# dell-research-harvard/effocr

Measured on AMD Instinct MI355X. Metric: glyph-crops/sec end-to-end (encode+kNN), 224x224 bs=1024, higher is better.
Workload: dtype bf16; 1 GPU; BASELINE configs[1]: vit_small_patch16_224 encoder (bf16 MFMA operands, fp32 accumulate/residual/LN/softmax), 1024x3x224x224 fp32 crops per GPU resident in HBM, 10000-row fp32 IndexFlatIP, k=10; seeded random-init weights; crops_per_gpu=1024, global_batch=1024, index_rows=10000, k=10, parallelism=1024 crops per GPU, weights+index replicated

## Files before the change

### effocr_amd/_lib.py

```python
import ctypes
import os
import subprocess
import threading

_HERE = os.path.dirname(os.path.abspath(__file__))
_CSRC = os.path.join(_HERE, "csrc")
SO_PATH = os.environ.get("EFFOCR_HIP_LIB") or os.path.join(_HERE, "libeffocr_hip.so")
SO_PATH_AB = os.path.join(_HERE, "libeffocr_hip_ab.so")

ABI_VERSION = 9
PREC = {"bf16": 0, "fp16": 1, "fp32": 2}
EPI = {"bias": 0, "bias_gelu": 1, "bias_resid": 2}

_lock = threading.Lock()
_lib = None
_loaded = {}


class EffOCRHipError(RuntimeError):
    pass


def build(force=False, verbose=False, ab=True):
    so = os.path.join(_HERE, "libeffocr_hip.so")
# ... 84 lines not shown
        "effocr_letterbox": (i32, [vp, i32, i32, i64, i32, i32, i32, i32, i32, i32, i32, f32p, vp]),
        "effocr_nms_workspace_bytes": (sz, [i32, i32]),
        "effocr_nms_batch_workspace_bytes": (sz, [i32, i32, i32]),
        "effocr_nms": (i32, [f32p, i32, i32, c.c_float, c.c_float, i32, i32, c.c_float, i32, f32p, vp, vp, sz, vp]),
        "effocr_nms_batch": (i32, [f32p, i32, i32, i32, c.c_float, c.c_float, i32, i32, c.c_float, i32, f32p, vp, vp, sz, vp]),
        "effocr_parse_char_boxes": (i32, [f32p, vp, i32, i32, i32, i32, i32, i32, f32p, vp, vp, vp, vp]),
        "effocr_op_linear": (i32, [i32, i32, vp, vp, f32p, f32p, vp, i32, i32, i32, vp]),
        "effocr_op_layernorm": (i32, [i32, f32p, i64, i32, f32p, f32p, c.c_float, vp, vp]),
        "effocr_op_attention": (i32, [i32, vp, vp, i32, i32, i32, vp]),
        "effocr_op_linear_blocked": (i32, [i32, i32, vp, vp, f32p, f32p, vp, i32, i32, i32, i32, vp]),
        "effocr_op_mlp_blocked": (i32, [i32, f32p, f32p, f32p, c.c_float, vp, f32p, vp, f32p, f32p, i32, i32, i32, i32, vp, sz, vp]),
        "effocr_op_mlp_ln_blocked": (i32, [i32, f32p, f32p, f32p, c.c_float, vp, f32p, vp, f32p, f32p, f32p, f32p, vp, i32, i32, i32, i32, vp, sz, vp]),
        "effocr_op_proj_mlp_blocked": (i32, [i32, f32p, vp, vp, f32p, f32p, f32p, c.c_float, vp, f32p, vp, f32p, f32p, i32, i32, i32, i32, vp, sz, vp]),
        "effocr_op_qkv_attn_blocked": (i32, [i32, vp, vp, f32p, vp, i32, i32, i32, i32, vp]),
        "effocr_op_layernorm_blocked": (i32, [i32, f32p, i64, i32, f32p, f32p, c.c_float, vp, vp]),
    }
    for name, (res, args) in sig.items():
        if os.environ.get("EFFOCR_HIP_LIB") and not hasattr(lib, name):
            def _absent(*a, _n=name, **k):
                raise EffOCRHipError(f"{_n} is not exported by the library EFFOCR_HIP_LIB points at")
            setattr(lib, name, _absent)
            continue
        fn = getattr(lib, name)
        fn.restype = res
        fn.argtypes = args
    return sig


EXPORTS = None

# ... 328 lines not shown
```

### effocr_amd/csrc/api.hip

```cpp
#include "../../include/effocr_hip.h"
#include "enc_core.hpp"


#include <math.h>
#include <algorithm>
#include <string.h>
#include <map>
#include <memory>
#include <string>
#include <vector>

namespace effocr {

namespace {

struct Param { std::string name; std::vector<int64_t> shape; int64_t numel; std::vector<float> data; bool set; };

struct VitCfg { int D, depth, heads, mlp; };
struct VitLayerOff { size_t ln1w, ln1b, qkvb, projb, ln2w, ln2b, fc1b, fc2b, qkvw, projw, fc1w, fc2w;
                     size_t qkvw_b, projw_b, fc1w_b, fc2w_b, projw_pp, fc2w_pp, projb_p, fc2b_p, qkvw_bv, qkvb_v;
                     size_t qkvw_bf, qkv_s, qkv_c, fc1w_bf, fc1_s, fc1_c; };
struct ConvSpec { std::string w, bn; int cin, cout, k, stride, pad; size_t w_off, b_off; };
struct CnxBlockOff { size_t dww, dwb, lnw, lnb, w1, b1, w2, b2, gamma; };
struct CnxStageOff { int C, Cp, depth; size_t dslnw, dslnb, dsw, dsb; std::vector<CnxBlockOff> blocks; };

}
}

using namespace effocr;

struct effocr_encoder {
  std::string arch;
  bool is_vit = false;
  int img = 224, prec = PREC_BF16, D = 0;
  std::vector<Param> params;
  std::map<std::string, int> index;
  VitCfg vit{};
  int T = 0, P = 0;
  size_t off_clspos0 = 0, off_pos = 0, off_patchb = 0, off_normw = 0, off_normb = 0, off_patchw = 0, off_patchw_b = 0;
  std::vector<VitLayerOff> layers;
  std::vector<ConvSpec> convs;
  bool is_cnx = false;
  std::vector<CnxStageOff> cnx;
  size_t cnx_stemw = 0, cnx_stemb = 0, cnx_stemlnw = 0, cnx_stemlnb = 0, cnx_headw = 0, cnx_headb = 0;
  bool is_mnv = false;
  MnvNet mnv{};
  size_t wbytes = 0;
  const char* wdev = nullptr;
  int debug = 0;
  int cls_only_last = 1;
  int mlp_stagger_min_rounds = 2;
  int mlp_tail_first = 96;
  int mlp_stagger = 2500;
  int use_projf = 1;
  int use_qkvattn = 1;
  int qa_min_batch = 1;
  int qa_hsplit = 0;
  int use_patchf = 1;
  int use_mlp = 1;
  int use_gemm3 = 1;
  int use_lnfold = 1;
  int tail_split = 1;
  int split6 = 1;
  int pair_parts = 1;
// ... 85 lines not shown
      L.fc2w_b = a.take((size_t)D * mlp * es);
      L.fc2w_pp = a.take((size_t)D * mlp * es);
      L.projw_pp = a.take((size_t)D * D * es);
      L.projb_p = a.take((size_t)D * 4);
      L.fc2b_p = a.take((size_t)D * 4);
      L.qkvw_bv = a.take((size_t)3 * D * D * es);
      L.qkvb_v = a.take((size_t)3 * D * 4);
      {
        L.qkvw_b = a.take((size_t)3 * D * D * es);
        L.projw_b = a.take((size_t)D * D * es);
        L.fc1w_b = a.take((size_t)mlp * D * es);
        L.qkvw_bf = a.take((size_t)3 * D * D * es); L.qkv_s = a.take((size_t)3 * D * 4); L.qkv_c = a.take((size_t)3 * D * 4);
        L.fc1w_bf = a.take((size_t)mlp * D * es); L.fc1_s = a.take((size_t)mlp * 4); L.fc1_c = a.take((size_t)mlp * 4);
      }
    }
  }
  e->wbytes = a.off;
}

void add_bn(effocr_encoder* e, const std::string& p, int c) {
  add_param(e, p + ".weight", {c}); add_param(e, p + ".bias", {c});
  add_param(e, p + ".running_mean", {c}); add_param(e, p + ".running_var", {c});
}

constexpr int CONV1_KPAD = 160;

void build_resnet18(effocr_encoder* e) {
  const int widths[4] = {64, 128, 256, 512};
  add_param(e, "conv1.weight", {64, 3, 7, 7});
  add_bn(e, "bn1", 64);
// ... 171 lines not shown
  float* cd = reinterpret_cast<float*>(blob.data() + c_off);
  for (int n = 0; n < N; ++n) {
    double ss = 0.0, cc = b[n];
    for (int k = 0; k < K; ++k) {
      const float v = W[(size_t)n * K + k] * gamma[k];
      wf[(size_t)n * K + k] = v;
      float r;
      if (prec == PREC_BF16) { const uint32_t u = (uint32_t)f32_to_bf16(v) << 16; memcpy(&r, &u, 4); }
      else r = (float)(_Float16)v;
      ss += (double)r;
      cc += (double)W[(size_t)n * K + k] * (double)beta[k];
    }
    sd[n] = (float)ss; cd[n] = (float)cc;
  }
  put_op_blocked(blob, w_off, wf.data(), N, K, prec);
}

void pack_vit(const effocr_encoder* e, std::vector<char>& blob) {
  const int D = e->vit.D;
  std::vector<float> cp(D);
  const auto& cls = P(e, "cls_token"); const auto& pos = P(e, "pos_embed");
  for (int d = 0; d < D; ++d) cp[d] = cls[d] + pos[d];
  put_f32(blob, e->off_clspos0, cp.data(), D);
  put_f32(blob, e->off_pos, pos.data(), pos.size());
  put_f32(blob, e->off_patchb, P(e, "patch_embed.proj.bias").data(), D);
  put_op(blob, e->off_patchw, P(e, "patch_embed.proj.weight").data(), (size_t)D * 768, e->prec);
  if (e->prec != PREC_FP32 && D % 32 == 0) put_op_blocked(blob, e->off_patchw_b, P(e, "patch_embed.proj.weight").data(), D, 768, e->prec);
  for (int i = 0; i < e->vit.depth; ++i) {
    const std::string p = "blocks." + std::to_string(i) + ".";
    const VitLayerOff& L = e->layers[i];
// ... 15 lines not shown
      put_op_blocked(blob, L.projw_pp, P(e, p + "attn.proj.weight").data(), D, D, e->prec, false, true);
      put_f32_rowperm(blob, L.projb_p, P(e, p + "attn.proj.bias").data(), D);
      put_f32_rowperm(blob, L.fc2b_p, P(e, p + "mlp.fc2.bias").data(), D);
      put_op_blocked(blob, L.qkvw_bv, P(e, p + "attn.qkv.weight").data(), 3 * D, D, e->prec, false, true, 2 * D);
      put_f32(blob, L.qkvb_v, P(e, p + "attn.qkv.bias").data(), 2 * (size_t)D);
      put_f32_rowperm(blob, L.qkvb_v + (size_t)2 * D * 4, P(e, p + "attn.qkv.bias").data() + 2 * D, D);
      {
        put_op_blocked(blob, L.qkvw_b, P(e, p + "attn.qkv.weight").data(), 3 * D, D, e->prec);
        put_op_blocked(blob, L.projw_b, P(e, p + "attn.proj.weight").data(), D, D, e->prec);
        put_op_blocked(blob, L.fc1w_b, P(e, p + "mlp.fc1.weight").data(), e->vit.mlp, D, e->prec);
        put_lnfold(blob, L.qkvw_bf, L.qkv_s, L.qkv_c, P(e, p + "attn.qkv.weight").data(), P(e, p + "attn.qkv.bias").data(),
                   P(e, p + "norm1.weight").data(), P(e, p + "norm1.bias").data(), 3 * D, D, e->prec);
        put_lnfold(blob, L.fc1w_bf, L.fc1_s, L.fc1_c, P(e, p + "mlp.fc1.weight").data(), P(e, p + "mlp.fc1.bias").data(),
                   P(e, p + "norm2.weight").data(), P(e, p + "norm2.bias").data(), e->vit.mlp, D, e->prec);
      }
    }
  }
  put_f32(blob, e->off_normw, P(e, "norm.weight").data(), D);
  put_f32(blob, e->off_normb, P(e, "norm.bias").data(), D);
}

void pack_resnet(const effocr_encoder* e, std::vector<char>& blob) {
  for (size_t ci = 0; ci < e->convs.size(); ++ci) {
    const ConvSpec& c = e->convs[ci];
    const auto& w = P(e, c.w);
    const auto& g = P(e, c.bn + ".weight"); const auto& bt = P(e, c.bn + ".bias");
    const auto& mu = P(e, c.bn + ".running_mean"); const auto& var = P(e, c.bn + ".running_var");
    const int K = c.k * c.k * c.cin;
    const int Kp = (ci == 0) ? CONV1_KPAD : K;
    float* wd = reinterpret_cast<float*>(blob.data() + c.w_off);
// ... 128 lines not shown
  }
  const int cls = prof_class(e, name);
  const size_t slot = e->prof_used++;
  const bool clk = e->prof_mode == 1 && slot < effocr_encoder::PROF_CLK_SLOTS &&
                   (e->prof_clk || hipMalloc(&e->prof_clk, effocr_encoder::PROF_CLK_SLOTS * 8192 * sizeof(unsigned long long)) == hipSuccess && hipMemset(e->prof_clk, 0, effocr_encoder::PROF_CLK_SLOTS * 8192 * sizeof(unsigned long long)) == hipSuccess);
  if (clk) (void)clock_sample(e->prof_clk + slot * 8192, s);
  (void)hipEventRecord(e->prof_pool[slot].first, s);
  const int rc = launch();
  (void)hipEventRecord(e->prof_pool[slot].second, s);
  if (clk) (void)clock_sample(e->prof_clk + slot * 8192 + 4096, s);
  e->prof_rec.push_back({cls, (int)slot});
  e->prof_work[cls] += work;
  return rc;
}

struct VitWs { size_t status, x, xn, qkv, att, h, stats, total, rows, hbytes; };
VitWs vit_ws(const effocr_encoder* e, int B) {
  const size_t M = align_up((size_t)B * e->T, 128), D = e->vit.D, es = prec_esize(e->prec);
  Alloc a; VitWs w;
  w.rows = M;
  w.status = a.take(256);
  w.x = a.take(M * D * 4);
  w.xn = a.take(M * D * es);
  w.qkv = a.take(M * 3 * D * es);
  w.att = a.take(M * D * es);
  size_t hb = M * e->vit.mlp * es, pb = (size_t)B * e->P * 768 * es;
  w.hbytes = hb > pb ? hb : pb;
  {
    const size_t cus = (size_t)device_cus(), np = M / 128, tail = np % cus;
    const size_t split = (tail && tail * 6 <= cus) ? 6 : (tail && tail * 4 <= cus) ? 4 : (tail && tail * 2 <= cus) ? 2 : 0;
// ... 12 lines not shown
  const char* wb = e->wdev;
  float* xs = reinterpret_cast<float*>(ws + w.x);
  void* xn = ws + w.xn; void* qkv = ws + w.qkv; void* att = ws + w.att; void* hb = ws + w.h;
  auto F = [&](size_t off) { return reinterpret_cast<const float*>(wb + off); };
  int rc;
  const double Md = (double)M, Dd = (double)D, Hd = (double)e->vit.mlp;
  const bool panel = e->use_panel && panel_gemm_supported(prec, 3 * D, D) && panel_gemm_supported(prec, e->vit.mlp, D);
  const bool g2 = e->use_gemm2 && gemm2_supported(prec, D, e->vit.mlp);
  const bool g2p = e->use_gemm2 && gemm2_supported(prec, D, 768);
  const bool g3all = !panel && e->use_gemm3 && gemm3_supported(prec, 3 * D, D) && gemm3_supported(prec, D, D) &&
                     gemm3_supported(prec, e->vit.mlp, D) && gemm3_supported(prec, D, e->vit.mlp);
  const int blk = (e->use_blocked && g2p && ((panel && g2) || g3all)) ? 1 : 0;
  const bool mlpf = blk && panel && e->use_mlp && mlp_fused_supported(prec, D, e->vit.mlp);
  const bool projf = mlpf && e->use_projf;
  const bool qaf = blk && panel && mlpf && qkv_attn_supported(prec, D, T) && (e->use_qkvattn == 2 || (e->use_qkvattn == 1 && (e->call_size_invariant || B >= e->qa_min_batch)));
  const bool g3 = blk && e->use_gemm3 && gemm3_supported(prec, D, e->vit.mlp);
  const bool patchf = blk && e->use_patchf && patch_embed_fused_supported(prec, D);
  if (!patchf && (rc = timed(e, "im2col_patch16", 0.0, s, [&] { return im2col_patch16(prec, x, x16, B, e->img, e->img, hb, s); }))) return rc;
  int* status = reinterpret_cast<int*>(ws + w.status);
  if (!patchf && (rc = set_cls_rows(F(e->off_clspos0), xs, B, T, D, blk, nullptr, s))) return rc;
  GemmArgs g{};
  if (patchf) {
    PatchArgs pa{};
    pa.x = x; pa.x16 = x16; pa.B = B; pa.H = e->img; pa.W = e->img; pa.Wb = wb + e->off_patchw_b; pa.bias = F(e->off_patchb); pa.pos = F(e->off_pos);
    pa.out = xs; pa.D = D; pa.P = Pn; pa.cls = F(e->off_clspos0);
    if ((rc = timed(e, "patch_embed_fused", 2.0 * B * Pn * Dd * 768.0, s, [&] { return patch_embed_fused(prec, pa, s); }))) return rc;
  } else {
  g.X = hb; g.ldx = 768; g.W = wb + e->off_patchw; g.ldw = 768; g.bias = F(e->off_patchb);
  g.out = xs; g.ldo = D; g.pos = F(e->off_pos); g.M = B * Pn; g.N = D; g.K = 768; g.P = Pn; g.blk_out = blk;
  if ((rc = timed(e, "gemm_patch_embed", 2.0 * B * Pn * Dd * 768.0, s, [&] { return g2p ? gemm2_nt(prec, EPI_PATCH, g, s) : gemm_nt(prec, EPI_PATCH, g, s); }))) return rc;
  }
  const float* cls_x = nullptr;
  bool xn_ready = false;
  for (int i = 0; i < e->vit.depth; ++i) {
    const VitLayerOff& L = e->layers[i];
    if (panel) {
      {
      PanelArgs p{};
      if (qaf) {
        if (!xn_ready && (rc = timed(e, "layernorm", 0.0, s, [&] { return layernorm_rows_blocked(prec, xs, M, D, F(L.ln1w), F(L.ln1b), 1e-6f, xn, s); }))) return rc;
        xn_ready = false;
        QkvAttnArgs q{};
        q.xn = xn; q.Wb = wb + L.qkvw_bv; q.bias = F(L.qkvb_v); q.out = att;
        q.B = B; q.T = T; q.D = D; q.rows_alloc = (int64_t)w.rows; q.hsplit = e->qa_hsplit;
        q.cls_only = (i + 1 == e->vit.depth && e->cls_only_last && projf) ? 1 : 0;
        const bool cls_k = q.cls_only && D == 384 && T > 192;
        const double qa_work = cls_k ? 2.0 * Md * 2.0 * Dd * Dd + 2.0 * (32.0 * B) * Dd * Dd + 4.0 * B * e->vit.heads * 32.0 * T * 64.0
                                     : 2.0 * Md * 3.0 * Dd * Dd + 4.0 * B * e->vit.heads * (double)T * T * 64.0;
        if ((rc = timed(e, "qkv_attn_fused", qa_work, s, [&] { return qkv_attn_fused(prec, q, s); }))) return rc;
      } else {
      p.A = xs; p.lda = D; p.gamma = F(L.ln1w); p.beta = F(L.ln1b); p.eps = 1e-6f; p.W = wb + L.qkvw; p.bias = F(L.qkvb);
      p.out = qkv; p.ldo = 3 * D; p.M = M; p.N = 3 * D; p.K = D; p.rows_padded = 1; p.debug = e->debug; p.panel_rows = e->panel_rows; p.no_tail_split = !e->tail_split;
      p.blk_a = blk; p.blk_out = blk;
      if ((rc = timed(e, "panel_ln_qkv", 2.0 * Md * 3.0 * Dd * Dd, s, [&] { return panel_gemm(prec, PRO_LN, EPI_BIAS, p, s); }))) return rc;
      if ((rc = timed(e, "attention", 4.0 * B * e->vit.heads * (double)T * T * 64.0, s, [&] { return attention(prec, qkv, att, B, T, e->vit.heads, blk, s); }))) return rc;
      }
      if (!projf) {
      p = PanelArgs{};
      p.A = att; p.lda = D; p.W = wb + L.projw; p.bias = F(L.projb); p.out = xs; p.ldo = D; p.resid = xs; p.ldr = D;
      p.M = M; p.N = D; p.K = D; p.rows_padded = 1; p.debug = e->debug; p.panel_rows = e->panel_rows; p.no_tail_split = !e->tail_split; p.blk_a = blk; p.blk_out = blk;
      if ((rc = timed(e, "panel_proj_resid", 2.0 * Md * Dd * Dd, s, [&] { return panel_gemm(prec, PRO_COPY, EPI_BIAS_RESID, p, s); }))) return rc;
      }
      }
      if (mlpf) {
        MlpArgs m{};
        m.x = xs; m.gamma = F(L.ln2w); m.beta = F(L.ln2b); m.eps = 1e-6f; m.W1b = wb + L.fc1w_b; m.b1 = F(L.fc1b);
        m.W2p = wb + L.fc2w_pp; m.b2 = F(L.fc2b_p); m.b2_logical = F(L.fc2b); m.M = M; m.D = D; m.H = e->vit.mlp; m.rows_alloc = (int)w.rows;
        m.partial = reinterpret_cast<float*>(hb); m.partial_bytes = w.hbytes; m.no_tail_split = !e->tail_split; m.no_split6 = !e->split6; m.pair = e->mlp_pair; m.no_pair_parts = !e->pair_parts; m.stagger = e->mlp_stagger; m.stagger_min_rounds = e->mlp_stagger_min_rounds; m.tail_first = e->mlp_tail_first;
        if (e->call_size_invariant) { m.no_tail_split = 1; m.pair = -1; }
        if (projf) {
          m.A = att; m.Wpp = wb + L.projw_pp; m.bp = F(L.projb_p);
          if (i + 1 == e->vit.depth && e->cls_only_last) {
            const size_t Bp = align_up((size_t)B, 128);
            float* xc = reinterpret_cast<float*>(qkv);
            void* ac = static_cast<char*>(qkv) + Bp * D * 4;
            if ((rc = timed(e, "gather_cls", 0.0, s, [&] { return gather_cls_rows_blocked(xs, att, B, T, D, xc, ac, s); }))) return rc;
            m.x = xc; m.A = ac; m.M = B; m.rows_alloc = (int)Bp;
            const double Bd = B;
            if ((rc = timed(e, "proj_mlp_cls", 4.0 * Bd * Hd * Dd + 2.0 * Bd * Dd * Dd, s, [&] { return mlp_fused(prec, m, s); }))) return rc;
            cls_x = xc;
            continue;
          }
          if (qaf && i + 1 < e->vit.depth) {
            m.xn_out = xn; m.gamma_n = F(e->layers[i + 1].ln1w); m.beta_n = F(e->layers[i + 1].ln1b);
            xn_ready = true;
          }
          if ((rc = timed(e, "proj_mlp_fused", 4.0 * Md * Hd * Dd + 2.0 * Md * Dd * Dd, s, [&] { return mlp_fused(prec, m, s); }))) return rc;
          continue;
        }
        if (qaf && i + 1 < e->vit.depth) {
          m.xn_out = xn; m.gamma_n = F(e->layers[i + 1].ln1w); m.beta_n = F(e->layers[i + 1].ln1b);
          xn_ready = true;
        }
// ... 387 lines not shown
  if (n == "debug") { enc->debug = value; return EFFOCR_OK; }
  if (n == "use_gemm2") { enc->use_gemm2 = value; return EFFOCR_OK; }
  if (n == "use_blocked") { enc->use_blocked = value; return EFFOCR_OK; }
  if (n == "tail_split") { enc->tail_split = value; return EFFOCR_OK; }
  if (n == "split6") { enc->split6 = value; return EFFOCR_OK; }
  if (n == "mlp_pair") { enc->mlp_pair = value; return EFFOCR_OK; }
  if (n == "pair_parts") { enc->pair_parts = value; return EFFOCR_OK; }
  if (n == "use_gemm3") { enc->use_gemm3 = value; return EFFOCR_OK; }
  if (n == "use_lnfold") { enc->use_lnfold = value; return EFFOCR_OK; }
  if (n == "use_mlp") { enc->use_mlp = value; return EFFOCR_OK; }
  if (n == "use_qkvattn") { enc->use_qkvattn = value; return EFFOCR_OK; }
  if (n == "qa_min_batch") { enc->qa_min_batch = value; return EFFOCR_OK; }
  if (n == "qa_hsplit") { enc->qa_hsplit = value; return EFFOCR_OK; }
  if (n == "use_patchf") { enc->use_patchf = value; return EFFOCR_OK; }
  if (n == "use_projf") { enc->use_projf = value; return EFFOCR_OK; }
  if (n == "cls_only_last") { enc->cls_only_last = value; return EFFOCR_OK; }
  if (n == "mlp_stagger_min_rounds") { enc->mlp_stagger_min_rounds = value < 1 ? 1 : value; return EFFOCR_OK; }
  if (n == "mlp_tail_first") { enc->mlp_tail_first = value < 0 ? 0 : value & ~7; return EFFOCR_OK; }
  if (n == "mlp_stagger") { enc->mlp_stagger = value < 0 ? 0 : value; return EFFOCR_OK; }
  if (n == "panel_rows") { if (value != 64 && value != 128) return fail(EFFOCR_EINVAL, "set_option: panel_rows must be 64 or 128"); enc->panel_rows = value; return EFFOCR_OK; }
  if (n == "call_size_invariant") {
    if (value != 0 && value != 1) return fail(EFFOCR_EINVAL, "set_option: call_size_invariant must be 0 or 1");
    enc->call_size_invariant = value; return EFFOCR_OK;
  }
  if (n == "chunk") { if (value < 0) return fail(EFFOCR_EINVAL, "set_option: chunk < 0"); enc->chunk = value; return EFFOCR_OK; }
  return fail(EFFOCR_EINVAL, "set_option: unknown option '" + n + "'");
}

int effocr_encoder_set_chunk(effocr_encoder_t* enc, int crops_per_chunk) {
  if (!enc || crops_per_chunk < 0) return fail(EFFOCR_EINVAL, "set_chunk: bad argument");
// ... 324 lines not shown
  a.M = m; a.D = d; a.H = h; a.rows_alloc = rows_alloc; a.partial = static_cast<float*>(scratch_dev); a.partial_bytes = scratch_bytes;
  return mlp_fused(precision, a, S(stream));
}

int effocr_op_qkv_attn_blocked(int precision, const void* xn_blk_dev, const void* wqkv_blk_dev, const float* bias_dev,
                               void* out_blk_dev, int batch, int tokens, int d, int rows_alloc, void* stream) {
  if (batch > 0 && (!xn_blk_dev || !wqkv_blk_dev || !bias_dev || !out_blk_dev))
    return fail(EFFOCR_EINVAL, "op_qkv_attn_blocked: NULL device pointer");
  if (batch < 0 || tokens < 1) return fail(EFFOCR_EINVAL, "op_qkv_attn_blocked: bad batch / tokens");
  QkvAttnArgs q{};
  q.xn = xn_blk_dev; q.Wb = wqkv_blk_dev; q.bias = bias_dev; q.out = out_blk_dev;
  q.B = batch; q.T = tokens; q.D = d; q.rows_alloc = rows_alloc;
  return qkv_attn_fused(precision, q, S(stream));
}

int effocr_op_layernorm_blocked(int out_precision, const float* x_blk_dev, int64_t rows, int d, const float* gamma_dev,
                                const float* beta_dev, float eps, void* out_blk_dev, void* stream) {
  if (rows > 0 && (!x_blk_dev || !gamma_dev || !beta_dev || !out_blk_dev)) return fail(EFFOCR_EINVAL, "op_layernorm_blocked: NULL device pointer");
  return layernorm_rows_blocked(out_precision, x_blk_dev, rows, d, gamma_dev, beta_dev, eps, out_blk_dev, S(stream));
}

int effocr_op_layernorm(int out_precision, const float* x_dev, int64_t rows, int d, const float* gamma_dev,
                        const float* beta_dev, float eps, void* out_dev, void* stream) {
  return layernorm_rows(out_precision, x_dev, rows, d, gamma_dev, beta_dev, eps, out_dev, S(stream));
}

int effocr_op_attention(int precision, const void* qkv_dev, void* out_dev, int batch, int tokens, int heads, void* stream) {
  return attention(precision, qkv_dev, out_dev, batch, tokens, heads, 0, S(stream));
}

// ... 2 lines not shown
```

### effocr_amd/csrc/kernels.hpp

```cpp
#pragma once
#include "common.hpp"

namespace effocr {

enum { PREC_BF16 = 0, PREC_FP16 = 1, PREC_FP32 = 2 };
enum { EPI_BIAS = 0, EPI_BIAS_GELU = 1, EPI_BIAS_RESID = 2, EPI_PATCH = 3,
       EPI_BIAS_SCALE_RESID = 4,
       EPI_BIAS_F32 = 5 };

static inline int prec_esize(int prec) { return prec == PREC_FP32 ? 4 : 2; }

struct GemmArgs {
  const void* X; int64_t ldx;
  const void* W; int64_t ldw;
  const float* bias;
  void* out; int64_t ldo;
  const float* resid; int64_t ldr;
  const float* pos;
  int M, N, K;
  int P;
  int blk_x;
  int blk_out;
  const void* Wblk;
  int rows_alloc;
// ... 35 lines not shown
int mlp_fused(int prec, const MlpArgs& a, hipStream_t s);

struct QkvAttnArgs {
  const void* xn;
  const void* Wb; const float* bias;
  void* out;
  int B, T, D;
  int64_t rows_alloc;
  int cls_only;
  int img0;
  int hsplit;
};
bool qkv_attn_supported(int prec, int D, int T);
int qkv_attn_fused(int prec, const QkvAttnArgs& a, hipStream_t s);

struct PatchArgs {
  const void* x; int B, H, W;
  int x16;
  const void* Wb;
  const float* bias; const float* pos;
  const float* cls;
  float* out;
  int D, P;
};
bool patch_embed_fused_supported(int prec, int D);
int patch_embed_fused(int prec, const PatchArgs& a, hipStream_t s);

enum { PRO_COPY = 0, PRO_LN = 1 };
struct PanelArgs {
  const void* A; int64_t lda;
// ... 114 lines not shown
```

### include/effocr_hip.h

```cpp
#ifndef EFFOCR_HIP_H
#define EFFOCR_HIP_H

#include <stddef.h>
#include <stdint.h>

#ifdef __cplusplus
extern "C" {
#endif

#define EFFOCR_ABI_VERSION 9

enum effocr_status {
  EFFOCR_OK = 0,
  EFFOCR_EINVAL = -1,
  EFFOCR_EUNSUPPORTED = -2,
  EFFOCR_EWORKSPACE = -3,
  EFFOCR_EHIP = -4,
  EFFOCR_ESTATE = -5,
  EFFOCR_EOVERFLOW = -6
};

enum effocr_precision {
  EFFOCR_PREC_BF16 = 0,
  EFFOCR_PREC_FP16 = 1,
// ... 114 lines not shown
                          int m, int d, int h, int rows_alloc, void* scratch_dev, size_t scratch_bytes, void* stream);
int effocr_op_mlp_ln_blocked(int precision, float* x_blk_dev, const float* gamma_dev, const float* beta_dev, float eps,
                             const void* w1_blk_dev, const float* b1_dev, const void* w2_perm_dev, const float* b2_perm_dev, const float* b2_dev,
                             const float* gamma_next_dev, const float* beta_next_dev, void* xn_blk_dev,
                             int m, int d, int h, int rows_alloc, void* scratch_dev, size_t scratch_bytes, void* stream);
int effocr_op_proj_mlp_blocked(int precision, float* x_blk_dev, const void* a_blk_dev, const void* wp_perm_dev, const float* bp_perm_dev,
                               const float* gamma_dev, const float* beta_dev, float eps, const void* w1_blk_dev, const float* b1_dev,
                               const void* w2_perm_dev, const float* b2_perm_dev, const float* b2_dev, int m, int d, int h, int rows_alloc,
                               void* scratch_dev, size_t scratch_bytes, void* stream);

int effocr_op_qkv_attn_blocked(int precision, const void* xn_blk_dev, const void* wqkv_blk_dev, const float* bias_dev,
                               void* out_blk_dev, int batch, int tokens, int d, int rows_alloc, void* stream);
int effocr_op_layernorm_blocked(int out_precision, const float* x_blk_dev, int64_t rows, int d, const float* gamma_dev,
                                const float* beta_dev, float eps, void* out_blk_dev, void* stream);

#ifdef __cplusplus
}
#endif
#endif
```

Baseline: 93720 glyph-crops/s.

## Compute last-layer CLS attention by folding K and V projections into query side

For the final ViT layer, where only the CLS token is needed, the new path skips the full K/V projection over all tokens. It computes q_cls·Wk per head (qt) and scores each token directly against the normalized input. It then forms the probability-weighted sum of inputs per head and applies Wv once per image. This removes the M×2D×D K/V GEMM on the last layer and replaces it with three custom kernels plus a specially packed weight copy. It is enabled by default for batches of at least 576 when call-size invariance is not requested, and it uses CUDA-core FMA rather than MFMA.

```diff
diff --git a/effocr_amd/_lib.py b/effocr_amd/_lib.py
--- a/effocr_amd/_lib.py
+++ b/effocr_amd/_lib.py
@@ -122,6 +122,9 @@
         "effocr_op_proj_mlp_blocked": (i32, [i32, f32p, vp, vp, f32p, f32p, f32p, c.c_float, vp, f32p, vp, f32p, f32p, i32, i32, i32, i32, vp, sz, vp]),
         "effocr_op_qkv_attn_blocked": (i32, [i32, vp, vp, f32p, vp, i32, i32, i32, i32, vp]),
         "effocr_op_layernorm_blocked": (i32, [i32, f32p, i64, i32, f32p, f32p, c.c_float, vp, vp]),
+        "effocr_op_cls_attn_pack_bytes": (sz, [i32]),
+        "effocr_op_cls_attn_pack": (i32, [i32, f32p, f32p, i32, vp, sz]),
+        "effocr_op_cls_attn": (i32, [i32, vp, vp, i32, i32, i32, i64, vp, vp, sz, vp]),
     }
     for name, (res, args) in sig.items():
         if os.environ.get("EFFOCR_HIP_LIB") and not hasattr(lib, name):
diff --git a/effocr_amd/csrc/api.hip b/effocr_amd/csrc/api.hip
--- a/effocr_amd/csrc/api.hip
+++ b/effocr_amd/csrc/api.hip
@@ -19,7 +19,8 @@
 struct VitCfg { int D, depth, heads, mlp; };
 struct VitLayerOff { size_t ln1w, ln1b, qkvb, projb, ln2w, ln2b, fc1b, fc2b, qkvw, projw, fc1w, fc2w;
                      size_t qkvw_b, projw_b, fc1w_b, fc2w_b, projw_pp, fc2w_pp, projb_p, fc2b_p, qkvw_bv, qkvb_v;
-                     size_t qkvw_bf, qkv_s, qkv_c, fc1w_bf, fc1_s, fc1_c; };
+                     size_t qkvw_bf, qkv_s, qkv_c, fc1w_bf, fc1_s, fc1_c;
+                     size_t cls_attn; };
 struct ConvSpec { std::string w, bn; int cin, cout, k, stride, pad; size_t w_off, b_off; };
 struct CnxBlockOff { size_t dww, dwb, lnw, lnb, w1, b1, w2, b2, gamma; };
 struct CnxStageOff { int C, Cp, depth; size_t dslnw, dslnb, dsw, dsb; std::vector<CnxBlockOff> blocks; };
@@ -48,6 +49,7 @@
   size_t wbytes = 0;
   const char* wdev = nullptr;
   int debug = 0;
+  int cls_attn_direct = 1;
   int cls_only_last = 1;
   int mlp_stagger_min_rounds = 2;
   int mlp_tail_first = 96;
@@ -163,6 +165,7 @@
         L.fc1w_bf = a.take((size_t)mlp * D * es); L.fc1_s = a.take((size_t)mlp * 4); L.fc1_c = a.take((size_t)mlp * 4);
       }
     }
+    if (cls_attn_supported(e->prec, D, e->T)) e->layers[depth - 1].cls_attn = a.take(cls_attn_pack_bytes(D));
   }
   e->wbytes = a.off;
 }
@@ -364,6 +367,20 @@
     sd[n] = (float)ss; cd[n] = (float)cc;
   }
   put_op_blocked(blob, w_off, wf.data(), N, K, prec);
+}
+
+void put_cls_attn(char* dst, const float* W, const float* b, int D, int prec) {
+  uint16_t* d = reinterpret_cast<uint16_t*>(dst);
+  const size_t dd = (size_t)D * D;
+  auto op = [&](float v) { return prec == PREC_FP16 ? f32_to_f16(v) : f32_to_bf16(v); };
+  for (int n = 0; n < D; ++n)
+    for (int k = 0; k < D; ++k) {
+      d[((size_t)(k >> 3) * D + n) * 8 + (k & 7)] = op(W[(size_t)n * D + k]);
+      d[dd + ((size_t)(n >> 3) * D + k) * 8 + (n & 7)] = op(W[dd + (size_t)n * D + k]);
+      d[2 * dd + ((size_t)(k >> 3) * D + n) * 8 + (k & 7)] = op(W[2 * dd + (size_t)n * D + k]);
+    }
+  memcpy(dst + 3 * dd * 2, b, (size_t)D * 4);
+  memcpy(dst + 3 * dd * 2 + (size_t)D * 4, b + 2 * D, (size_t)D * 4);
 }
 
 void pack_vit(const effocr_encoder* e, std::vector<char>& blob) {
@@ -409,6 +426,7 @@
         put_lnfold(blob, L.fc1w_bf, L.fc1_s, L.fc1_c, P(e, p + "mlp.fc1.weight").data(), P(e, p + "mlp.fc1.bias").data(),
                    P(e, p + "norm2.weight").data(), P(e, p + "norm2.bias").data(), e->vit.mlp, D, e->prec);
       }
+      if (L.cls_attn) put_cls_attn(blob.data() + L.cls_attn, P(e, p + "attn.qkv.weight").data(), P(e, p + "attn.qkv.bias").data(), D, e->prec);
     }
   }
   put_f32(blob, e->off_normw, P(e, "norm.weight").data(), D);
@@ -567,6 +585,8 @@
   return rc;
 }
 
+constexpr int CLS_ATTN_MIN_BATCH = 576;
+
 struct VitWs { size_t status, x, xn, qkv, att, h, stats, total, rows, hbytes; };
 VitWs vit_ws(const effocr_encoder* e, int B) {
   const size_t M = align_up((size_t)B * e->T, 128), D = e->vit.D, es = prec_esize(e->prec);
@@ -609,6 +629,9 @@
   const bool mlpf = blk && panel && e->use_mlp && mlp_fused_supported(prec, D, e->vit.mlp);
   const bool projf = mlpf && e->use_projf;
   const bool qaf = blk && panel && mlpf && qkv_attn_supported(prec, D, T) && (e->use_qkvattn == 2 || (e->use_qkvattn == 1 && (e->call_size_invariant || B >= e->qa_min_batch)));
+  const bool cls_direct = qaf && projf && e->cls_only_last && e->layers[e->vit.depth - 1].cls_attn != 0 &&
+                          (e->cls_attn_direct == 2 || (e->cls_attn_direct == 1 && !e->call_size_invariant && B >= CLS_ATTN_MIN_BATCH));
+  ClsAttnArgs ca{};
   const bool g3 = blk && e->use_gemm3 && gemm3_supported(prec, D, e->vit.mlp);
   const bool patchf = blk && e->use_patchf && patch_embed_fused_supported(prec, D);
   if (!patchf && (rc = timed(e, "im2col_patch16", 0.0, s, [&] { return im2col_patch16(prec, x, x16, B, e->img, e->img, hb, s); }))) return rc;
@@ -639,10 +662,18 @@
         q.xn = xn; q.Wb = wb + L.qkvw_bv; q.bias = F(L.qkvb_v); q.out = att;
         q.B = B; q.T = T; q.D = D; q.rows_alloc = (int64_t)w.rows; q.hsplit = e->qa_hsplit;
         q.cls_only = (i + 1 == e->vit.depth && e->cls_only_last && projf) ? 1 : 0;
+        if (q.cls_only && cls_direct) {
+          ca.xn = xn; ca.packed = wb + L.cls_attn; ca.B = B; ca.T = T; ca.D = D; ca.rows_alloc = (int64_t)w.rows;
+          ca.qt = reinterpret_cast<float*>(att); ca.m = ca.qt + (size_t)B * e->vit.heads * D;
+          const double Bd = B;
+          if ((rc = timed(e, "cls_attn_q", 4.0 * Bd * Dd * Dd, s, [&] { return cls_attn_q(prec, ca, s); }))) return rc;
+          if ((rc = timed(e, "cls_attn", 4.0 * Md * e->vit.heads * Dd, s, [&] { return cls_attn_rows(prec, ca, s); }))) return rc;
+        } else {
         const bool cls_k = q.cls_only && D == 384 && T > 192;
         const double qa_work = cls_k ? 2.0 * Md * 2.0 * Dd * Dd + 2.0 * (32.0 * B) * Dd * Dd + 4.0 * B * e->vit.heads * 32.0 * T * 64.0
                                      : 2.0 * Md * 3.0 * Dd * Dd + 4.0 * B * e->vit.heads * (double)T * T * 64.0;
         if ((rc = timed(e, "qkv_attn_fused", qa_work, s, [&] { return qkv_attn_fused(prec, q, s); }))) return rc;
+        }
       } else {
       p.A = xs; p.lda = D; p.gamma = F(L.ln1w); p.beta = F(L.ln1b); p.eps = 1e-6f; p.W = wb + L.qkvw; p.bias = F(L.qkvb);
       p.out = qkv; p.ldo = 3 * D; p.M = M; p.N = 3 * D; p.K = D; p.rows_padded = 1; p.debug = e->debug; p.panel_rows = e->panel_rows; p.no_tail_split = !e->tail_split;
@@ -669,9 +700,12 @@
             const size_t Bp = align_up((size_t)B, 128);
             float* xc = reinterpret_cast<float*>(qkv);
             void* ac = static_cast<char*>(qkv) + Bp * D * 4;
-            if ((rc = timed(e, "gather_cls", 0.0, s, [&] { return gather_cls_rows_blocked(xs, att, B, T, D, xc, ac, s); }))) return rc;
+            const double Bd = B;
+            if (qaf && cls_direct) {
+              ca.x = xs; ca.xc = xc; ca.ac = ac;
+              if ((rc = timed(e, "cls_attn_v", 2.0 * Bd * Dd * Dd, s, [&] { return cls_attn_v(prec, ca, s); }))) return rc;
+            } else if ((rc = timed(e, "gather_cls", 0.0, s, [&] { return gather_cls_rows_blocked(xs, att, B, T, D, xc, ac, s); }))) return rc;
             m.x = xc; m.A = ac; m.M = B; m.rows_alloc = (int)Bp;
-            const double Bd = B;
             if ((rc = timed(e, "proj_mlp_cls", 4.0 * Bd * Hd * Dd + 2.0 * Bd * Dd * Dd, s, [&] { return mlp_fused(prec, m, s); }))) return rc;
             cls_x = xc;
             continue;
@@ -1089,6 +1123,10 @@
   if (n == "qa_hsplit") { enc->qa_hsplit = value; return EFFOCR_OK; }
   if (n == "use_patchf") { enc->use_patchf = value; return EFFOCR_OK; }
   if (n == "use_projf") { enc->use_projf = value; return EFFOCR_OK; }
+  if (n == "cls_attn_direct") {
+    if (value < 0 || value > 2) return fail(EFFOCR_EINVAL, "set_option: cls_attn_direct must be 0, 1 or 2");
+    enc->cls_attn_direct = value; return EFFOCR_OK;
+  }
   if (n == "cls_only_last") { enc->cls_only_last = value; return EFFOCR_OK; }
   if (n == "mlp_stagger_min_rounds") { enc->mlp_stagger_min_rounds = value < 1 ? 1 : value; return EFFOCR_OK; }
   if (n == "mlp_tail_first") { enc->mlp_tail_first = value < 0 ? 0 : value & ~7; return EFFOCR_OK; }
@@ -1443,6 +1481,30 @@
   return qkv_attn_fused(precision, q, S(stream));
 }
 
+size_t effocr_op_cls_attn_pack_bytes(int d) { return d > 0 && d % 8 == 0 ? cls_attn_pack_bytes(d) : 0; }
+
+int effocr_op_cls_attn_pack(int precision, const float* wqkv_host, const float* bqkv_host, int d, void* packed_host, size_t packed_bytes) {
+  if (!wqkv_host || !bqkv_host || !packed_host) return fail(EFFOCR_EINVAL, "op_cls_attn_pack: NULL argument");
+  if (precision != PREC_BF16 && precision != PREC_FP16) return fail(EFFOCR_EUNSUPPORTED, "op_cls_attn_pack: 16-bit precisions only");
+  if (d <= 0 || d % 8) return fail(EFFOCR_EINVAL, "op_cls_attn_pack: embed dim must be a positive multiple of 8");
+  if (packed_bytes < cls_attn_pack_bytes(d)) return fail(EFFOCR_EWORKSPACE, "op_cls_attn_pack: output buffer too small");
+  put_cls_attn(static_cast<char*>(packed_host), wqkv_host, bqkv_host, d, precision);
+  return EFFOCR_OK;
+}
+
+int effocr_op_cls_attn(int precision, const void* xn_blk_dev, const void* packed_dev, int batch, int tokens, int d, int64_t rows_alloc,
+                       void* out_blk_dev, void* scratch_dev, size_t scratch_bytes, void* stream) {
+  if (batch < 0 || tokens < 1) return fail(EFFOCR_EINVAL, "op_cls_attn: bad batch / tokens");
+  if (batch > 0 && (!xn_blk_dev || !packed_dev || !out_blk_dev || !scratch_dev)) return fail(EFFOCR_EINVAL, "op_cls_attn: NULL device pointer");
+  if (scratch_bytes < cls_attn_scratch_bytes(batch)) return fail(EFFOCR_EWORKSPACE, "op_cls_attn: scratch too small");
+  ClsAttnArgs a{};
+  a.xn = xn_blk_dev; a.packed = packed_dev; a.B = batch; a.T = tokens; a.D = d; a.rows_alloc = rows_alloc;
+  a.qt = static_cast<float*>(scratch_dev); a.m = a.qt + cls_attn_scratch_bytes(batch) / 8; a.ac = out_blk_dev;
+  int rc;
+  if ((rc = cls_attn_q(precision, a, S(stream))) || (rc = cls_attn_rows(precision, a, S(stream)))) return rc;
+  return cls_attn_v(precision, a, S(stream));
+}
+
 int effocr_op_layernorm_blocked(int out_precision, const float* x_blk_dev, int64_t rows, int d, const float* gamma_dev,
                                 const float* beta_dev, float eps, void* out_blk_dev, void* stream) {
   if (rows > 0 && (!x_blk_dev || !gamma_dev || !beta_dev || !out_blk_dev)) return fail(EFFOCR_EINVAL, "op_layernorm_blocked: NULL device pointer");
diff --git a/effocr_amd/csrc/cls_attn.hip b/effocr_amd/csrc/cls_attn.hip
--- /dev/null
+++ b/effocr_amd/csrc/cls_attn.hip
@@ -0,0 +1,302 @@
+#include "kernels.hpp"
+
+namespace effocr {
+namespace {
+
+constexpr int CA_D = 384, CA_H = 6, CA_NCH = CA_D / 8, CA_IMG = 4;
+constexpr int CA_ROWS_THREADS = 1024, CA_WAVES = CA_ROWS_THREADS / 64;
+constexpr int CA_QT_BYTES = CA_H * CA_D * 4;
+constexpr int CA_RED_BYTES = CA_WAVES * CA_H * CA_D * 4;
+constexpr float CA_SCALE = 0.125f * 1.44269504088896340736f;
+
+typedef float f32x2 __attribute__((ext_vector_type(2)));
+typedef float f32x4e __attribute__((ext_vector_type(4)));
+
+template <typename E>
+__global__ __launch_bounds__(CA_D) void cls_attn_q_kernel(const char* __restrict__ xn, const u32x4* __restrict__ pq, const u32x4* __restrict__ pk,
+                                                          const float* __restrict__ bq, float* __restrict__ qt, int B, int T) {
+  __shared__ f32x4e n0[CA_D];
+  __shared__ f32x4e qs[CA_D];
+  const int t = threadIdx.x, img0 = blockIdx.x * CA_IMG;
+  {
+    f32x4e v = {0.f, 0.f, 0.f, 0.f};
+#pragma unroll
+    for (int i = 0; i < CA_IMG; ++i)
+      if (img0 + i < B) v[i] = unpack1<E>(*reinterpret_cast<const uint32_t*>(xn + blk_off((int64_t)(img0 + i) * T, t >> 3, CA_NCH) + (t & 6) * 2), t & 1);
+    n0[t] = v;
+  }
+  __syncthreads();
+  f32x2 a = {0.f, 0.f}, b = {0.f, 0.f};
+#pragma unroll 4
+  for (int kc = 0; kc < CA_D / 8; ++kc) {
+    const u32x4 w = pq[kc * CA_D + t];
+#pragma unroll
+    for (int e = 0; e < 8; ++e) {
+      const float wf = unpack1<E>(w[e >> 1], e & 1);
+      const f32x4e nv = n0[8 * kc + e];
+      a = __builtin_elementwise_fma(f32x2{wf, wf}, f32x2{nv[0], nv[1]}, a);
+      b = __builtin_elementwise_fma(f32x2{wf, wf}, f32x2{nv[2], nv[3]}, b);
+    }
+  }
+  const float bias = bq[t];
+  qs[t] = f32x4e{a[0] + bias, a[1] + bias, b[0] + bias, b[1] + bias};
+  __syncthreads();
+  for (int h = 0; h < CA_H; ++h) {
+    a = f32x2{0.f, 0.f}; b = f32x2{0.f, 0.f};
+#pragma unroll 4
+    for (int dc = 0; dc < 8; ++dc) {
+      const u32x4 w = pk[(8 * h + dc) * CA_D + t];
+#pragma unroll
+      for (int e = 0; e < 8; ++e) {
+        const float wf = unpack1<E>(w[e >> 1], e & 1);
+        const f32x4e qv = qs[64 * h + 8 * dc + e];
+        a = __builtin_elementwise_fma(f32x2{wf, wf}, f32x2{qv[0], qv[1]}, a);
+        b = __builtin_elementwise_fma(f32x2{wf, wf}, f32x2{qv[2], qv[3]}, b);
+      }
+    }
+    const float r[CA_IMG] = {a[0], a[1], b[0], b[1]};
+#pragma unroll
+    for (int i = 0; i < CA_IMG; ++i)
+      if (img0 + i < B) qt[((int64_t)(img0 + i) * CA_H + h) * CA_D + t] = r[i] * CA_SCALE;
+  }
+}
+
+template <typename E>
+__global__ __launch_bounds__(CA_D) void cls_attn_v_kernel(const float* __restrict__ m, const u32x4* __restrict__ pv, const float* __restrict__ bv,
+                                                          const char* __restrict__ x, char* __restrict__ xc, char* __restrict__ ac, int B, int T) {
+  __shared__ f32x4e ms[CA_H * CA_D];
+  const int t = threadIdx.x, img0 = blockIdx.x * CA_IMG;
+  for (int idx = t; idx < CA_H * CA_D; idx += CA_D) {
+    f32x4e v = {0.f, 0.f, 0.f, 0.f};
+#pragma unroll
+    for (int i = 0; i < CA_IMG; ++i)
+      if (img0 + i < B) v[i] = m[(int64_t)(img0 + i) * CA_H * CA_D + idx];
+    ms[idx] = v;
+  }
+  __syncthreads();
+  const f32x4e* mh = ms + (t >> 6) * CA_D;
+  f32x2 a = {0.f, 0.f}, b = {0.f, 0.f};
+#pragma unroll 4
+  for (int cc = 0; cc < CA_D / 8; ++cc) {
+    const u32x4 w = pv[cc * CA_D + t];
+#pragma unroll
+    for (int e = 0; e < 8; ++e) {
+      const float wf = unpack1<E>(w[e >> 1], e & 1);
+      const f32x4e mv = mh[8 * cc + e];
+      a = __builtin_elementwise_fma(f32x2{wf, wf}, f32x2{mv[0], mv[1]}, a);
+      b = __builtin_elementwise_fma(f32x2{wf, wf}, f32x2{mv[2], mv[3]}, b);
+    }
+  }
+  const float bias = bv[t];
+  const float r[CA_IMG] = {a[0] + bias, a[1] + bias, b[0] + bias, b[1] + bias};
+#pragma unroll
+  for (int i = 0; i < CA_IMG; ++i) {
+    const int img = img0 + i;
+    if (img >= B) break;
+    *reinterpret_cast<E*>(ac + blk_off(img, t >> 3, CA_NCH) + (t & 7) * 2) = (E)r[i];
+    if (xc) *reinterpret_cast<float*>(xc + blk_off(img, t >> 2, CA_D / 4) + (t & 3) * 4) =
+                *reinterpret_cast<const float*>(x + blk_off((int64_t)img * T, t >> 2, CA_D / 4) + (t & 3) * 4);
+  }
+}
+
+template <typename E>
+__global__ __launch_bounds__(CA_ROWS_THREADS) void cls_attn_rows_kernel(const char* __restrict__ xn, const float* __restrict__ qt, float* __restrict__ m, int T,
+                                                                        int rows_bytes) {
+  extern __shared__ __attribute__((aligned(16))) char smem[];
+  char* rows = smem;
+  float* qs = reinterpret_cast<float*>(smem + rows_bytes);
+  const int t = threadIdx.x, lane = t & 63, w = wave_id(), img = blockIdx.x;
+  {
+    u32x4 buf[3][4];
+#pragma unroll
+    for (int ci = 0; ci < 3; ++ci)
+#pragma unroll
+      for (int i = 0; i < 4; ++i) {
+        const int j = lane + 64 * i;
+        if (j < T) buf[ci][i] = *reinterpret_cast<const u32x4*>(xn + blk_off((int64_t)img * T + j, w + CA_WAVES * ci, CA_NCH));
+      }
+    for (int idx = t; idx < CA_H * CA_D; idx += CA_ROWS_THREADS) qs[idx] = qt[(int64_t)img * CA_H * CA_D + idx];
+#pragma unroll
+    for (int ci = 0; ci < 3; ++ci)
+#pragma unroll
+      for (int i = 0; i < 4; ++i) {
+        const int j = lane + 64 * i;
+        if (j < T) *reinterpret_cast<u32x4*>(rows + j * 768 + ((w + CA_WAVES * ci + j) % CA_NCH) * 16) = buf[ci][i];
+      }
+  }
+  __syncthreads();
+  float sc[CA_H];
+  const int r = w * 16 + (lane & 15);
+  {
+    const int rc = r < T ? r : T - 1, rr = rc % CA_NCH, c0 = (lane >> 4) * 12;
+    f32x2 acc[CA_H];
+#pragma unroll
+    for (int h = 0; h < CA_H; ++h) acc[h] = f32x2{0.f, 0.f};
+#pragma unroll 2
+    for (int ci = 0; ci < 12; ++ci) {
+      const int c = c0 + ci;
+      int ph = c + rr; ph = ph >= CA_NCH ? ph - CA_NCH : ph;
+      const u32x4 d = *reinterpret_cast<const u32x4*>(rows + rc * 768 + ph * 16);
+      f32x2 f[4];
+#pragma unroll
+      for (int e = 0; e < 4; ++e) f[e] = f32x2{unpack1<E>(d[e], 0), unpack1<E>(d[e], 1)};
+#pragma unroll
+      for (int h = 0; h < CA_H; ++h) {
+        const f32x4e q0 = *reinterpret_cast<const f32x4e*>(qs + h * CA_D + c * 8), q1 = *reinterpret_cast<const f32x4e*>(qs + h * CA_D + c * 8 + 4);
+        acc[h] = __builtin_elementwise_fma(f[0], f32x2{q0[0], q0[1]}, acc[h]);
+        acc[h] = __builtin_elementwise_fma(f[1], f32x2{q0[2], q0[3]}, acc[h]);
+        acc[h] = __builtin_elementwise_fma(f[2], f32x2{q1[0], q1[1]}, acc[h]);
+        acc[h] = __builtin_elementwise_fma(f[3], f32x2{q1[2], q1[3]}, acc[h]);
+      }
+    }
+#pragma unroll
+    for (int h = 0; h < CA_H; ++h) {
+      float s = acc[h][0] + acc[h][1];
+      s += __shfl_xor(s, 16);
+      s += __shfl_xor(s, 32);
+      sc[h] = s;
+    }
+  }
+  __syncthreads();
+  float* ps = qs;
+  if (lane < 16 && r < T) {
+    *reinterpret_cast<f32x4e*>(ps + r * 8) = f32x4e{sc[0], sc[1], sc[2], sc[3]};
+    *reinterpret_cast<f32x2*>(ps + r * 8 + 4) = f32x2{sc[4], sc[5]};
+  }
+  __syncthreads();
+  if (w < CA_H) {
+    float s[4], mx = -INFINITY;
+#pragma unroll
+    for (int i = 0; i < 4; ++i) {
+      const int j = lane + 64 * i;
+      s[i] = j < T ? ps[j * 8 + w] : -INFINITY;
+      mx = fmaxf(mx, s[i]);
+    }
+#pragma unroll
+    for (int o = 1; o < 64; o <<= 1) mx = fmaxf(mx, __shfl_xor(mx, o));
+    float sum = 0.f;
+#pragma unroll
+    for (int i = 0; i < 4; ++i) {
+      const int j = lane + 64 * i;
+      s[i] = j < T ? __builtin_amdgcn_exp2f(s[i] - mx) : 0.f;
+      sum += s[i];
+    }
+#pragma unroll
+    for (int o = 1; o < 64; o <<= 1) sum += __shfl_xor(sum, o);
+    const float inv = 1.0f / sum;
+#pragma unroll
+    for (int i = 0; i < 4; ++i) {
+      const int j = lane + 64 * i;
+      if (j < T) ps[j * 8 + w] = s[i] * inv;
+    }
+  }
+  __syncthreads();
+  f32x2 acc[CA_H][3];
+#pragma unroll
+  for (int h = 0; h < CA_H; ++h)
+#pragma unroll
+    for (int i = 0; i < 3; ++i) acc[h][i] = f32x2{0.f, 0.f};
+  for (int j = w; j < T; j += CA_WAVES) {
+    const int rr = j % CA_NCH;
+    const f32x4e p0 = *reinterpret_cast<const f32x4e*>(ps + j * 8);
+    const f32x2 p1 = *reinterpret_cast<const f32x2*>(ps + j * 8 + 4);
+    const float p[CA_H] = {p0[0], p0[1], p0[2], p0[3], p1[0], p1[1]};
+#pragma unroll
+    for (int i = 0; i < 3; ++i) {
+      int ph = ((lane + 64 * i) >> 2) + rr; ph = ph >= CA_NCH ? ph - CA_NCH : ph;
+      const uint32_t d = *reinterpret_cast<const uint32_t*>(rows + j * 768 + ph * 16 + (lane & 3) * 4);
+      const f32x2 f = {unpack1<E>(d, 0), unpack1<E>(d, 1)};
+#pragma unroll
+      for (int h = 0; h < CA_H; ++h) acc[h][i] = __builtin_elementwise_fma(f32x2{p[h], p[h]}, f, acc[h][i]);
+    }
+  }
+  __syncthreads();
+  f32x2* red = reinterpret_cast<f32x2*>(smem);
+#pragma unroll
+  for (int h = 0; h < CA_H; ++h)
+#pragma unroll
+    for (int i = 0; i < 3; ++i) red[(w * CA_H + h) * (CA_D / 2) + lane + 64 * i] = acc[h][i];
+  __syncthreads();
+  const float* redf = reinterpret_cast<const float*>(smem);
+  for (int idx = t; idx < CA_H * CA_D; idx += CA_ROWS_THREADS) {
+    float s = redf[idx];
+#pragma unroll
+    for (int k = 1; k < CA_WAVES; ++k) s += redf[k * CA_H * CA_D + idx];
+    m[(int64_t)img * CA_H * CA_D + idx] = s;
+  }
+}
+
+int rows_lds(int T, int* rows_bytes) {
+  *rows_bytes = T * 768 > CA_RED_BYTES ? T * 768 : CA_RED_BYTES;
+  return *rows_bytes + CA_QT_BYTES;
+}
+
+template <typename E>
+int launch_rows(const ClsAttnArgs& a, hipStream_t s) {
+  int rows_bytes;
+  const int lds = rows_lds(a.T, &rows_bytes);
+  static bool attr_set = false;
+  if (!attr_set) {
+    if (hipFuncSetAttribute(reinterpret_cast<const void*>(&cls_attn_rows_kernel<E>), hipFuncAttributeMaxDynamicSharedMemorySize, 160 * 1024) != hipSuccess)
+      return fail(EFFOCR_EHIP, "cls_attn: hipFuncSetAttribute(MaxDynamicSharedMemorySize) failed");
+    attr_set = true;
+  }
+  hipLaunchKernelGGL((cls_attn_rows_kernel<E>), dim3((unsigned)a.B), dim3(CA_ROWS_THREADS), (size_t)lds, s, static_cast<const char*>(a.xn), a.qt, a.m, a.T,
+                     rows_bytes);
+  return check_launch("cls_attn");
+}
+
+}
+
+size_t cls_attn_pack_bytes(int D) { return (size_t)3 * D * D * 2 + (size_t)2 * D * 4; }
+size_t cls_attn_scratch_bytes(int B) { return (size_t)2 * B * CA_H * CA_D * 4; }
+
+bool cls_attn_supported(int prec, int D, int T) {
+  int rb;
+  return (prec == PREC_BF16 || prec == PREC_FP16) && D == CA_D && T >= 1 && T <= 256 && rows_lds(T, &rb) <= 160 * 1024;
+}
+
+static int cls_attn_check(int prec, const ClsAttnArgs& a) {
+  if (!cls_attn_supported(prec, a.D, a.T)) return fail(EFFOCR_EUNSUPPORTED, "cls_attn: needs a 16-bit precision, embed dim 384 and at most 201 tokens");
+  if (a.B < 0 || a.rows_alloc < (int64_t)a.B * a.T) return fail(EFFOCR_EINVAL, "cls_attn: bad batch / rows_alloc");
+  return EFFOCR_OK;
+}
+
+template <typename E>
+int launch_q(const ClsAttnArgs& a, hipStream_t s) {
+  const char* pk = static_cast<const char*>(a.packed);
+  const size_t dd = (size_t)CA_D * CA_D * 2;
+  hipLaunchKernelGGL((cls_attn_q_kernel<E>), dim3((unsigned)((a.B + CA_IMG - 1) / CA_IMG)), dim3(CA_D), 0, s, static_cast<const char*>(a.xn),
+                     reinterpret_cast<const u32x4*>(pk), reinterpret_cast<const u32x4*>(pk + dd), reinterpret_cast<const float*>(pk + 3 * dd), a.qt, a.B, a.T);
+  return check_launch("cls_attn_q");
+}
+
+template <typename E>
+int launch_v(const ClsAttnArgs& a, hipStream_t s) {
+  const char* pk = static_cast<const char*>(a.packed);
+  const size_t dd = (size_t)CA_D * CA_D * 2;
+  hipLaunchKernelGGL((cls_attn_v_kernel<E>), dim3((unsigned)((a.B + CA_IMG - 1) / CA_IMG)), dim3(CA_D), 0, s, a.m, reinterpret_cast<const u32x4*>(pk + 2 * dd),
+                     reinterpret_cast<const float*>(pk + 3 * dd) + CA_D, reinterpret_cast<const char*>(a.x), reinterpret_cast<char*>(a.xc),
+                     static_cast<char*>(a.ac), a.B, a.T);
+  return check_launch("cls_attn_v");
+}
+
+int cls_attn_q(int prec, const ClsAttnArgs& a, hipStream_t s) {
+  if (int rc = cls_attn_check(prec, a)) return rc;
+  if (a.B == 0) return EFFOCR_OK;
+  return prec == PREC_BF16 ? launch_q<__bf16>(a, s) : launch_q<_Float16>(a, s);
+}
+
+int cls_attn_rows(int prec, const ClsAttnArgs& a, hipStream_t s) {
+  if (int rc = cls_attn_check(prec, a)) return rc;
+  if (a.B == 0) return EFFOCR_OK;
+  return prec == PREC_BF16 ? launch_rows<__bf16>(a, s) : launch_rows<_Float16>(a, s);
+}
+
+int cls_attn_v(int prec, const ClsAttnArgs& a, hipStream_t s) {
+  if (int rc = cls_attn_check(prec, a)) return rc;
+  if (a.B == 0) return EFFOCR_OK;
+  return prec == PREC_BF16 ? launch_v<__bf16>(a, s) : launch_v<_Float16>(a, s);
+}
+
+}
diff --git a/effocr_amd/csrc/kernels.hpp b/effocr_amd/csrc/kernels.hpp
--- a/effocr_amd/csrc/kernels.hpp
+++ b/effocr_amd/csrc/kernels.hpp
@@ -73,6 +73,22 @@
 bool qkv_attn_supported(int prec, int D, int T);
 int qkv_attn_fused(int prec, const QkvAttnArgs& a, hipStream_t s);
 
+struct ClsAttnArgs {
+  const void* xn;
+  const void* packed;
+  int B, T, D;
+  int64_t rows_alloc;
+  float* qt; float* m;
+  const float* x; float* xc;
+  void* ac;
+};
+bool cls_attn_supported(int prec, int D, int T);
+size_t cls_attn_pack_bytes(int D);
+size_t cls_attn_scratch_bytes(int B);
+int cls_attn_q(int prec, const ClsAttnArgs& a, hipStream_t s);
+int cls_attn_rows(int prec, const ClsAttnArgs& a, hipStream_t s);
+int cls_attn_v(int prec, const ClsAttnArgs& a, hipStream_t s);
+
 struct PatchArgs {
   const void* x; int B, H, W;
   int x16;
diff --git a/include/effocr_hip.h b/include/effocr_hip.h
--- a/include/effocr_hip.h
+++ b/include/effocr_hip.h
@@ -152,6 +152,11 @@
 int effocr_op_layernorm_blocked(int out_precision, const float* x_blk_dev, int64_t rows, int d, const float* gamma_dev,
                                 const float* beta_dev, float eps, void* out_blk_dev, void* stream);
 
+size_t effocr_op_cls_attn_pack_bytes(int d);
+int effocr_op_cls_attn_pack(int precision, const float* wqkv_host, const float* bqkv_host, int d, void* packed_host, size_t packed_bytes);
+int effocr_op_cls_attn(int precision, const void* xn_blk_dev, const void* packed_dev, int batch, int tokens, int d, int64_t rows_alloc,
+                       void* out_blk_dev, void* scratch_dev, size_t scratch_bytes, void* stream);
+
 #ifdef __cplusplus
 }
 #endif
```

Result: no change. 94650 glyph-crops/s (median of 6 runs) (+1.0%).
